# minyoungg/pix2latent

Measured on AMD Instinct MI355X. Metric: candidate-latent evals/sec (fwd+loss+bwd), BigGAN-256 pop=18, higher is better.
Workload: dtype f32 (fp32 tensors everywhere; convolutions >= 32x32 and the self-attention multiply on the 16-bit MFMA pipe with fp32-grade operand splits and fp32 accumulate: the 16x16 Winograd, direct and sub-pixel 3x3 kernels and the 1x1 kernels (4x4 layers included) on power-of-two scaled operands in 2 fp16 pie

## Files before the change

### include/p2l.h

```cpp
#ifndef P2L_H_
#define P2L_H_

#include <stddef.h>
#include <stdint.h>

#ifdef __cplusplus
extern "C" {
#endif

#define P2L_OK 0
#define P2L_EINVAL (-1)
#define P2L_ELAUNCH (-2)
#define P2L_EWS (-3)
#define P2L_EUNSUP (-4)

int p2l_version(void);
const char* p2l_strerror(int rc);
int p2l_last_hip_error(void);


enum { P2L_ACT_NONE = 0, P2L_ACT_RELU = 1, P2L_ACT_TANH = 2,
       P2L_ACT_LRELU_SQRT2 = 3  };
enum { P2L_POOL_NONE = 0, P2L_POOL_MAX = 1, P2L_POOL_SUM = 2 };
enum { P2L_PRO_NONE = 0, P2L_PRO_AFFINE_RELU = 1, P2L_PRO_AFFINE = 2 };
// ... 110 lines not shown
       P2L_WFMT_FLAG_ATTN_GEMM = 0x40,
       P2L_WFMT_FLAG_NO_AMAX = 0x80
                                       };
int p2l_pack_conv_weight_bf3t(const float* w_oihw, int O, int I, int N_pad, int K_pad,
                              int transpose_flip, float* w_packed, void* stream);
int p2l_pack_conv_weight_pw(const float* w_oihw, int O, int I, int N_pad, int K_pad,
                            int transpose_flip, float* w_packed, void* stream);
size_t p2l_packed_weight_floats(int taps, int N_pad, int K_pad, int wfmt);
enum {
  P2L_FORM_AUTO = 0,
  P2L_FORM_NO_WINO = 1,
  P2L_FORM_WINO_ANY = 2,
  P2L_FORM_WINO_8X16 = 4,
  P2L_FORM_NO_PW = 8,
  P2L_FORM_NO_THIN = 16,
  P2L_FORM_WINO_BF3 = 32,
  P2L_FORM_WINO_H2_8X16 = 64,
  P2L_FORM_WINO_H2_16X16 = 128,
  P2L_FORM_NO_H2R = 256,
  P2L_FORM_H2R_SEQ_EPI = 512,
  P2L_FORM_NO_SP_SKIP = 1024,
  P2L_FORM_NO_SP_PAIR = 2048,
  P2L_FORM_SP_PAIR = 4096,
  P2L_FORM_GENERIC_EPI = 8192
};
int p2l_conv_epilogue_class(const P2LConv* d, const P2LConvExtra* ex, const P2LArb* arb, const float* bias,
                            const float* res, const float* mask, const float* y, const float* yp,
                            const void* workspace, size_t ws_bytes);
int p2l_wino_split_factor(int H, int W, int Cin, int Cout);
int p2l_pack_conv_weight_bf3w(const float* w_oihw, int O, int I, int taps, int N_pad,
                              int K_pad, int transpose_flip, float* w_packed, void* stream);
int p2l_pack_conv_weight_bf3(const float* w_oihw, int O, int I, int taps, int N_pad,
                             int K_pad, int transpose_flip, float* w_packed, void* stream);
int p2l_pack_conv_weight_subpix_bf3(const float* w_oihw, int O, int I, int N_pad, int K_pad,
                                    int transpose_flip, int mode, float* w_packed,
                                    void* stream);
size_t p2l_packed_subpix_weight_floats(int N_pad, int K_pad, int wfmt);
int p2l_pack_conv_weight_subpix_h2(const float* w_oihw, int O, int I, int N_pad, int K_pad,
                                   int transpose_flip, int mode, float* w_packed, void* stream);

typedef struct P2LGemm {
  int32_t batch, M, N, K;
  int32_t lda, ldb, ldc;
  int64_t stride_a, stride_b, stride_c;
  int32_t a_kmajor, b_kmajor;
  float alpha;
  int32_t accumulate;
// ... 7 lines not shown
typedef struct P2LAttn {
  int32_t B, Nq, Nk, d, dv;
} P2LAttn;
int p2l_attn_supported(const P2LAttn* d);
size_t p2l_attn_fwd_ws_bytes(const P2LAttn* d);
int p2l_attn_fwd(const P2LAttn* d, const float* q, const float* k, const float* v, float* out,
                 float* lse, void* ws, size_t ws_bytes, void* stream);
size_t p2l_attn_bwd_dv_ws_bytes(const P2LAttn* d);
int p2l_attn_bwd_dv(const P2LAttn* d, const float* q, const float* k, const float* dout,
                    const float* lse, float* dv, void* ws, size_t ws_bytes, void* stream);
size_t p2l_attn_bwd_qk_ws_bytes(const P2LAttn* d);
int p2l_attn_bwd_qk(const P2LAttn* d, const float* q, const float* k, const float* v,
                    const float* out, const float* dout, const float* lse, float* dst, float* dq,
                    float* dk, void* ws, size_t ws_bytes, void* stream);

int p2l_linear_fwd(const float* x, const float* W, const float* bias, float* y,
                   int Bn, int K, int N, void* stream);
int p2l_linear_bwd(const float* dy, const float* W, float* dx, int Bn, int K,
                   int N, int accumulate, void* stream);
int p2l_linear_fwd_ld(const float* x, int x_ld, const float* W, const float* bias, float* y,
                      int Bn, int K, int N, void* stream);
int p2l_linear_bwd_ld(const float* dy, const float* W, float* dx, int dx_ld, int Bn, int K,
                      int N, int accumulate, void* stream);

int p2l_cbn_fold_fwd(const float* g_raw, const float* b_raw, const float* mean,
                     const float* rstd, float* s, float* t, int Bn, int C,
                     int raw_ld, void* stream);
int p2l_cbn_fold_bwd(const float* ds, const float* dt, const float* mean,
                     const float* rstd, float* dg_raw, float* db_raw, int Bn,
                     int C, int raw_ld, void* stream);

int p2l_affine_relu_bwd_nblk(int P);
int p2l_affine_relu_bwd(const float* da, int da_ld, const float* x, int x_ld,
                        const float* s, const float* t, int st_bstride,
                        const float* skip, int skip_ld, int skip_C, int skip_ups,
                        float* dx, int dx_ld, float* ds, float* dt,
                        int dsdt_bstride, float* partial, int Bn, int H, int W,
                        int C, void* stream);

int p2l_scale_bwd(const float* da, int da_ld, const float* x, int x_ld, const float* s,
                  int st_bstride, const float* skip, int skip_ld, int skip_C, float* dx,
                  int dx_ld, float* ds, float* dt_scratch, int dsdt_bstride, float* partial,
                  int Bn, int H, int W, int C, void* stream);

int p2l_softmax_fwd(const float* S, float* P, int64_t rows, int cols,
                    void* stream);
// ... 391 lines not shown
```

### pix2latent_amd/_native.py

```python
import ctypes as C
import os

import torch

_HERE = os.path.dirname(os.path.abspath(__file__))
LIB_PATH = os.environ.get('P2L_LIB_PATH') or os.path.join(_HERE, 'libp2l_hip.so')

c_float_p = C.c_void_p


class P2LConv(C.Structure):
    _fields_ = [('B', C.c_int32), ('H', C.c_int32), ('W', C.c_int32),
                ('Cin', C.c_int32), ('Cout', C.c_int32), ('taps', C.c_int32),
                ('ups', C.c_int32), ('x_ld', C.c_int32), ('pro', C.c_int32),
                ('pro_bstride', C.c_int32), ('alpha', C.c_float), ('act', C.c_int32),
                ('pool', C.c_int32), ('y_ld', C.c_int32), ('yp_ld', C.c_int32),
                ('n_store', C.c_int32), ('res_ld', C.c_int32), ('res_ups', C.c_int32),
                ('mask_ld', C.c_int32), ('splitk', C.c_int32), ('ext', C.c_int32),
                ('wfmt', C.c_int32), ('form', C.c_int32), ('algo_flops', C.c_double),
                ('w_floats', C.c_int64)]


class P2LAmax(C.Structure):
    _fields_ = [('out', C.c_void_p), ('outp', C.c_void_p), ('in_', C.c_void_p), ('in_n', C.c_int32),
# ... 123 lines not shown


def prof_totals():
    t = P2LProfTotals()
    t.size = C.sizeof(P2LProfTotals)
    check(lib().p2l_prof_totals(C.byref(t)), 'p2l_prof_totals')
    return t


prof_end = prof_totals


ACT_NONE, ACT_RELU, ACT_TANH, ACT_LRELU_SQRT2 = 0, 1, 2, 3
WFMT_F32, WFMT_BF16X3, WFMT_BF16X3W, WFMT_PW, WFMT_BF16X3T = 0, 1, 2, 3, 4
WFMT_FLAG_PW, WFMT_FLAG_THIN, WFMT_FLAG_ATTN_GEMM, WFMT_FLAG_NO_AMAX = 0x10, 0x20, 0x40, 0x80
FORM_AUTO, FORM_NO_WINO, FORM_WINO_ANY, FORM_WINO_8X16, FORM_NO_PW, FORM_NO_THIN, FORM_WINO_BF3 = 0, 1, 2, 4, 8, 16, 32
FORM_WINO_H2_8X16, FORM_WINO_H2_16X16 = 64, 128
FORM_H2R_SEQ_EPI = 512
FORM_NO_SP_SKIP = 1024
FORM_NO_SP_PAIR = 2048
FORM_SP_PAIR = 4096
FORM_NO_H2R = 256
FORM_GENERIC_EPI = 8192


def default_wfmt():
    v = os.environ.get('P2L_CONV_WFMT', 'bf16x3').lower()
    if v in ('f32', 'fp32', '0'):
        return WFMT_F32
    if v in ('bf16x3-direct', 'bf3d', '1'):
        return WFMT_BF16X3
    if v in ('bf16x3', 'bf3', 'bf16x3w', '2'):
        return WFMT_BF16X3W
    raise ValueError('P2L_CONV_WFMT=%r (expected f32, bf16x3 or bf16x3-direct)' % v)


def default_thin():
    return os.environ.get('P2L_THIN', '1') != '0' and default_wfmt() != WFMT_F32


def default_attn_gemm():
    return os.environ.get('P2L_ATTN', '1') == '0'


def default_no_amax():
    return os.environ.get('P2L_AMAX', '1') == '0'
# ... 45 lines not shown

POOL_NONE, POOL_MAX, POOL_SUM = 0, 1, 2
PRO_NONE, PRO_AFFINE_RELU, PRO_AFFINE = 0, 1, 2

EXPORTS = [
    'p2l_version', 'p2l_strerror', 'p2l_last_hip_error',
    'p2l_conv_workspace_bytes', 'p2l_conv_amax_slots', 'p2l_conv_epilogue_class', 'p2l_selftest_amaxreg', 'p2l_conv_suggest_splitk', 'p2l_conv_fwd', 'p2l_conv_fwd_ex',
    'p2l_pack_conv_weight', 'p2l_pack_conv_weight_subpix', 'p2l_pack_conv_weight_bf3',
    'p2l_pack_conv_weight_bf3w', 'p2l_packed_weight_floats', 
    'p2l_pack_conv_weight_bf3t',
    'p2l_pack_conv_weight_pw', 'p2l_adam_step_dev',
    'p2l_attn_supported', 'p2l_attn_fwd_ws_bytes', 'p2l_attn_fwd', 'p2l_attn_bwd_dv_ws_bytes',
    'p2l_attn_bwd_dv', 'p2l_attn_bwd_qk_ws_bytes', 'p2l_attn_bwd_qk',
    'p2l_pack_conv_weight_subpix_bf3', 'p2l_pack_conv_weight_subpix_h2', 'p2l_packed_subpix_weight_floats', 'p2l_gemm', 'p2l_gemm_ws_bytes', 'p2l_gemm_ws', 'p2l_linear_fwd', 'p2l_linear_bwd',
    'p2l_cbn_fold_fwd', 'p2l_cbn_fold_bwd', 'p2l_affine_relu_bwd_nblk',
    'p2l_affine_relu_bwd', 'p2l_softmax_fwd', 'p2l_softmax_bwd', 'p2l_maxpool2_bwd', 'p2l_maxpool2_bwd_amax', 'p2l_maxpool2_bwd_amax_slots',
    'p2l_relu_mask', 'p2l_nchw3_to_nhwc16', 'p2l_nhwc16_to_nchw3', 'p2l_tanh_bwd16',
    'p2l_weight_sum', 'p2l_weight_map', 'p2l_l1_loss_nblk', 'p2l_l1_loss_fwd',
    'p2l_l1_loss_bwd', 'p2l_lpips_normalize', 'p2l_lpips_tap_nblk', 'p2l_lpips_tap_fwd',
    'p2l_lpips_tap_bwd', 'p2l_lpips_tap_pool_bwd', 'p2l_bilinear_adjoint', 'p2l_reduce_rows', 'p2l_adam_step',
    'p2l_clamp', 'p2l_affine_grid_sample', 'p2l_affine_grid_sample_bwd', 'p2l_affine_grid_sample_bwd_ws_bytes', 'p2l_vec_scale_div', 'p2l_concat2', 'p2l_split2',
    'p2l_biggan_ws_bytes', 'p2l_biggan_fwd', 'p2l_biggan_bwd', 'p2l_biggan_ws_lookup',
    'p2l_loss_cache_floats', 'p2l_projloss_ws_bytes', 'p2l_projloss_ws_lookup', 'p2l_projloss_prepare',
    'p2l_projloss_fwd', 'p2l_projloss_bwd', 'p2l_mfma_probe', 'p2l_prof_begin', 'p2l_prof_totals', 'p2l_prof_step', 'p2l_prof_dump', 'p2l_wino_split_factor', 'p2l_linear_fwd_ld', 'p2l_linear_bwd_ld', 'p2l_scale_bwd',
    'p2l_sg2_pixelnorm_fwd', 'p2l_sg2_pixelnorm_bwd', 'p2l_sg2_bias_lrelu_fwd', 'p2l_sg2_lrelu_bwd',
    'p2l_sg2_demod_fwd', 'p2l_sg2_demod_bwd', 'p2l_sg2_blur_fwd', 'p2l_sg2_act_bwd_nblk',
    'p2l_sg2_styled_act_bwd', 'p2l_sg2_blur_bwd', 'p2l_sg2_rgb_up_fwd', 'p2l_sg2_rgb_up_bwd',
    'p2l_sg2_clamp16_fwd', 'p2l_sg2_clamp16_bwd', 'p2l_broadcast_rows', 'p2l_add_inplace',
    'p2l_sg2_ws_bytes', 'p2l_sg2_ws_lookup', 'p2l_sg2_synthesis_fwd', 'p2l_sg2_synthesis_bwd', 'p2l_sg2_mapping_fwd',
    'p2l_sg2_mapping_bwd', 'p2l_conv_arb_fusable', 'p2l_conv_arb_nblk',
    'p2l_conv_dgrad_arb', 'p2l_conv_arb_split_fusable', 'p2l_conv_arb_nblk_ws',
    'p2l_conv_dgrad_arb_ws', 'p2l_arb_finish', 'p2l_arb_defer_begin', 'p2l_arb_defer_flush',
    'p2l_arb_defer_cancel',
    'p2l_gconv_fwd', 'p2l_maxpool3s2_fwd', 'p2l_maxpool3s2_bwd', 'p2l_conv1_dgrad',
    'p2l_alex_cache_floats', 'p2l_alexloss_ws_bytes', 'p2l_alexloss_prepare', 'p2l_alexloss_fwd',
    'p2l_alexloss_bwd',
    'p2l_pack_gconv_weight', 'p2l_sqz_cache_floats', 'p2l_sqzloss_ws_bytes', 'p2l_sqzloss_prepare', 'p2l_sqzloss_fwd',
    'p2l_sqzloss_bwd', 'p2l_sqzloss_ws_lookup',
    'p2l_sg2_blur_fwd_amax', 'p2l_sg2_styled_act_bwd_amax', 'p2l_sg2_blur_bwd_amax', 'p2l_sg2_noise_relayout',
    'p2l_sg2_rows_defer_begin', 'p2l_sg2_rows_defer_flush', 'p2l_sg2_rows_defer_cancel',
    'p2l_color_adjust_ws_bytes', 'p2l_color_adjust',
    'p2l_gram_f64_ws_bytes', 'p2l_gram_f64', 'p2l_gram_f64_wide_ws_bytes', 'p2l_gram_f64_wide',
    'p2l_poisson_blend_ws_bytes', 'p2l_poisson_blend',
    'p2l_sg2_noise_reg_ws_bytes', 'p2l_sg2_noise_reg_fwd', 'p2l_sg2_noise_reg_bwd', 'p2l_sg2_noise_normalize',
    'p2l_area_pool3_to_nhwc16', 'p2l_area_pool_nchw', 'p2l_area_unpool16_add_nchw3',
    'p2l_latent_prior_ws_bytes', 'p2l_latent_prior_fwd', 'p2l_latent_prior_bwd',
    'p2l_l2_loss_nblk', 'p2l_l2_loss_fwd', 'p2l_l2_loss_bwd', 'p2l_adam_step_sched',
# ... 124 lines not shown
```

### pix2latent_amd/csrc/p2l_ops.hip

```cpp
#include "p2l_common.h"

namespace {

__device__ __forceinline__ float block_sum_256(float v, float* red ) {
  v = wave_sum(v);
  const int lane = threadIdx.x & 63, wave = threadIdx.x >> 6;
  __syncthreads();
  if (lane == 0) red[wave] = v;
  __syncthreads();
  return (red[0] + red[1]) + (red[2] + red[3]);
}

template <int BG>
__global__ __launch_bounds__(256) void linear_fwd_kernel(
    const float* __restrict__ x, const float* __restrict__ W,
    const float* __restrict__ bias, float* __restrict__ y, int Bn, int b_begin,
    int K, int N, int x_ld) {
  extern __shared__ float sm[];
  float* xs = sm;
  float* red = sm + BG * K;
  const int tid = threadIdx.x, nl = tid & 63, kg = tid >> 6;
  const int n = blockIdx.x * 64 + nl;
  const int nb = min(BG, Bn - b_begin);
  for (int i = tid; i < BG * K; i += 256) {
// ... 9 lines not shown
  if (n < N) {
#pragma unroll 8
    for (int kk = k0; kk < k0 + kper; ++kk) {
      const float w = W[(size_t)kk * N + n];
#pragma unroll
      for (int b = 0; b < BG; ++b) acc[b] = fmaf(xs[b * K + kk], w, acc[b]);
    }
  }
#pragma unroll
  for (int b = 0; b < BG; ++b) red[(kg * BG + b) * 64 + nl] = acc[b];
  __syncthreads();
  for (int i = tid; i < BG * 64; i += 256) {
    const int b = i >> 6, c = i & 63;
    const int nn = blockIdx.x * 64 + c;
    if (b < nb && nn < N) {
      float v = (red[(0 * BG + b) * 64 + c] + red[(1 * BG + b) * 64 + c]) +
                (red[(2 * BG + b) * 64 + c] + red[(3 * BG + b) * 64 + c]);
      if (bias) v += bias[nn];
      y[(size_t)(b_begin + b) * N + nn] = v;
    }
  }
}

template <int BG>
__global__ __launch_bounds__(1024) void linear_bwd_kernel(
    const float* __restrict__ dy, const float* __restrict__ W,
    float* __restrict__ dx, int Bn, int b_begin, int K, int N, int accumulate, int dx_ld) {
  __shared__ float red[BG][16];
  const int k = blockIdx.x, tid = threadIdx.x;
  const int nb = min(BG, Bn - b_begin);
  float acc[BG];
#pragma unroll
  for (int b = 0; b < BG; ++b) acc[b] = 0.f;
  const float* wrow = W + (size_t)k * N;
  const int N4 = N >> 2;
  for (int i = tid; i < N4; i += 1024) {
    const f32x4 w = *reinterpret_cast<const f32x4*>(wrow + 4 * i);
#pragma unroll
    for (int b = 0; b < BG; ++b) {
      if (b < nb) {
        const f32x4 d = *reinterpret_cast<const f32x4*>(dy + (size_t)(b_begin + b) * N + 4 * i);
        acc[b] += (d.x * w.x + d.y * w.y) + (d.z * w.z + d.w * w.w);
      }
    }
  }
  for (int n = 4 * N4 + tid; n < N; n += 1024) {
    const float w = wrow[n];
#pragma unroll
    for (int b = 0; b < BG; ++b)
      if (b < nb) acc[b] = fmaf(dy[(size_t)(b_begin + b) * N + n], w, acc[b]);
  }
  const int lane = tid & 63, wave = tid >> 6;
#pragma unroll
  for (int b = 0; b < BG; ++b) {
    const float v = wave_sum(acc[b]);
    if (lane == 0) red[b][wave] = v;
  }
  __syncthreads();
  if (tid < nb) {
    float s = 0.f;
#pragma unroll
    for (int w = 0; w < 16; ++w) s += red[tid][w];
    float* p = dx + (size_t)(b_begin + tid) * dx_ld + k;
    *p = accumulate ? (*p + s) : s;
  }
}

__global__ void cbn_fold_fwd_kernel(const float* g_raw, const float* b_raw,
                                    const float* mean, const float* rstd,
                                    float* s, float* t, int Bn, int C, int raw_ld) {
  const int i = blockIdx.x * 256 + threadIdx.x;
  if (i >= Bn * C) return;
  const int b = i / C, c = i - b * C;
  const float gain = 1.f + g_raw[(size_t)b * raw_ld + c];
  const float bias = b_raw[(size_t)b * raw_ld + c];
  const float sv = gain * rstd[c];
  s[i] = sv;
  t[i] = bias - mean[c] * sv;
}

__global__ void cbn_fold_bwd_kernel(const float* ds, const float* dt,
                                    const float* mean, const float* rstd,
                                    float* dg_raw, float* db_raw, int Bn, int C,
                                    int raw_ld) {
  const int i = blockIdx.x * 256 + threadIdx.x;
  if (i >= Bn * C) return;
// ... 797 lines not shown
  if (!x || !W || !y || K < 4 || K % 4 || K > 1024 || Bn < 1 || N < 1 || x_ld < K) return P2L_EINVAL;
  constexpr int BG = 16, BGW = 24;
  const size_t lds = (size_t)(BG * K + 4 * BG * 64) * sizeof(float);
  const size_t ldsw = (size_t)(BGW * K + 4 * BGW * 64) * sizeof(float);
  if (cdiv(Bn, BGW) < cdiv(Bn, BG) && ldsw <= 64 * 1024) {
    for (int b0 = 0; b0 < Bn; b0 += BGW)
      hipLaunchKernelGGL(linear_fwd_kernel<BGW>, dim3(cdiv(N, 64)), dim3(256), ldsw,
                         ST(stream), x, W, bias, y, Bn, b0, K, N, x_ld);
    return p2l_check_launch();
  }
  for (int b0 = 0; b0 < Bn; b0 += BG) {
    hipLaunchKernelGGL(linear_fwd_kernel<BG>, dim3(cdiv(N, 64)), dim3(256), lds,
                       ST(stream), x, W, bias, y, Bn, b0, K, N, x_ld);
  }
  return p2l_check_launch();
}

extern "C" int p2l_linear_bwd_ld(const float* dy, const float* W, float* dx, int dx_ld, int Bn,
                                 int K, int N, int accumulate, void* stream);
extern "C" int p2l_linear_bwd(const float* dy, const float* W, float* dx, int Bn,
                              int K, int N, int accumulate, void* stream) {
  return p2l_linear_bwd_ld(dy, W, dx, K, Bn, K, N, accumulate, stream);
}
extern "C" int p2l_linear_bwd_ld(const float* dy, const float* W, float* dx, int dx_ld, int Bn,
                                 int K, int N, int accumulate, void* stream) {
  if (!dy || !W || !dx || Bn < 1 || K < 1 || N < 4 || (N % 4) || dx_ld < K) return P2L_EINVAL;
  constexpr int BG = 16, BGW = 24;
  if (cdiv(Bn, BGW) < cdiv(Bn, BG)) {
    for (int b0 = 0; b0 < Bn; b0 += BGW)
      hipLaunchKernelGGL(linear_bwd_kernel<BGW>, dim3(K), dim3(1024), 0, ST(stream), dy,
                         W, dx, Bn, b0, K, N, accumulate, dx_ld);
    return p2l_check_launch();
  }
  for (int b0 = 0; b0 < Bn; b0 += BG)
    hipLaunchKernelGGL(linear_bwd_kernel<BG>, dim3(K), dim3(1024), 0, ST(stream), dy,
                       W, dx, Bn, b0, K, N, accumulate, dx_ld);
  return p2l_check_launch();
}

extern "C" int p2l_cbn_fold_fwd(const float* g_raw, const float* b_raw,
                                const float* mean, const float* rstd, float* s,
                                float* t, int Bn, int C, int raw_ld, void* stream) {
  if (!g_raw || !b_raw || !mean || !rstd || !s || !t) return P2L_EINVAL;
  if (Bn < 1 || C < 1 || raw_ld < C || (int64_t)Bn * C > INT32_MAX) return P2L_EINVAL;
  hipLaunchKernelGGL(cbn_fold_fwd_kernel, dim3(cdiv(Bn * C, 256)), dim3(256), 0,
                     ST(stream), g_raw, b_raw, mean, rstd, s, t, Bn, C, raw_ld);
  return p2l_check_launch();
}
extern "C" int p2l_cbn_fold_bwd(const float* ds, const float* dt, const float* mean,
                                const float* rstd, float* dg_raw, float* db_raw,
                                int Bn, int C, int raw_ld, void* stream) {
  if (!ds || !dt || !mean || !rstd || !dg_raw || !db_raw) return P2L_EINVAL;
  if (Bn < 1 || C < 1 || raw_ld < C || (int64_t)Bn * C > INT32_MAX) return P2L_EINVAL;
  hipLaunchKernelGGL(cbn_fold_bwd_kernel, dim3(cdiv(Bn * C, 256)), dim3(256), 0,
                     ST(stream), ds, dt, mean, rstd, dg_raw, db_raw, Bn, C, raw_ld);
  return p2l_check_launch();
}

extern "C" int p2l_affine_relu_bwd_nblk(int P) { return cdiv(P, ARB_SLAB); }

// ... 381 lines not shown
```

### pix2latent_amd/csrc/p2l_pw.hip

```cpp
#include "p2l_conv_k.h"
#include <type_traits>

#include <atomic>

using namespace p2lconv;

namespace {

template <int KS> struct PwCfg {
  static constexpr int SUB = KS / 16;
  static constexpr int A_FLOATS = SUB * 128 * 24;
  static constexpr int B_FLOATS = SUB * 64 * 24;
  static constexpr size_t LDS_BYTES = (size_t)(A_FLOATS + B_FLOATS) * sizeof(float);
};

__device__ __forceinline__ void pw_store_split(float* As, int row, int q4, const f32x4 x) {
  bf16x4 ph, pm, pl;
  split3(x, ph, pm, pl);
  char* rb = reinterpret_cast<char*>(As) + row * 96 + (q4 & 1) * 8;
  char* rq = rb + bf3_chunk(q4 >> 1, row) * 16;
  *reinterpret_cast<bf16x4*>(rq) = ph;
  *reinterpret_cast<bf16x4*>(rq + 32) = pm;
  *reinterpret_cast<bf16x4*>(rq + 64) = pl;
}
// ... 105 lines not shown
        f32x16 t = acc[j];
        t = __builtin_amdgcn_mfma_f32_32x32x16_bf16(a3, b1, t, 0, 0, 0);
        t = __builtin_amdgcn_mfma_f32_32x32x16_bf16(a1, b3, t, 0, 0, 0);
        t = __builtin_amdgcn_mfma_f32_32x32x16_bf16(a2, b2, t, 0, 0, 0);
        t = __builtin_amdgcn_mfma_f32_32x32x16_bf16(a2, b1, t, 0, 0, 0);
        t = __builtin_amdgcn_mfma_f32_32x32x16_bf16(a1, b2, t, 0, 0, 0);
        t = __builtin_amdgcn_mfma_f32_32x32x16_bf16(a1, b1, t, 0, 0, 0);
        acc[j] = t;
      }
    }
    __syncthreads();
    if (more) write_lds();
    __syncthreads();
  }
  epilogue_vec<2>(k, acc, smem, wave, lane, b0, y0, x0, n0, tile_in_image, 0, 0, 0);
}


constexpr int PWH_SUB = 2;
constexpr int PWH_A_FLOATS = PWH_SUB * 128 * 16, PWH_B_FLOATS = PWH_SUB * 64 * 16;
constexpr int PWH_EPI_FLOATS = 4 * 32 * (64 + 4);
constexpr size_t PWH_LDS_BYTES =
    (size_t)(PWH_A_FLOATS + PWH_B_FLOATS > PWH_EPI_FLOATS ? PWH_A_FLOATS + PWH_B_FLOATS : PWH_EPI_FLOATS) * sizeof(float);
__device__ __forceinline__ int h2_chunk(int c, int row) { return c ^ ((row >> 2) & 3); }
__device__ __forceinline__ int h2_chunk_a(int c, int row, int sub) { return h2_chunk(c, row) ^ ((sub & 1) << 1); }
__device__ __forceinline__ void pw_store_split_h2(float* As, int row, int q4, int sub, const f32x4 x) {
  const h16x4 h = __builtin_convertvector(x, h16x4);
  const f32x4 w = __builtin_convertvector(h, f32x4);
  const h16x4 m = __builtin_convertvector(x - w, h16x4);
  char* rb = reinterpret_cast<char*>(As) + row * 64 + (q4 & 1) * 8;
  *reinterpret_cast<h16x4*>(rb + h2_chunk_a(q4 >> 1, row, sub) * 16) = h;
  *reinterpret_cast<h16x4*>(rb + h2_chunk_a(2 + (q4 >> 1), row, sub) * 16) = m;
}

#ifndef P2L_PW_ABL
#define P2L_PW_ABL 0
#endif
template <int PRO, bool SM = false, int EC = EPI_GENERIC>
__global__ __launch_bounds__(256, SM ? 3 : 4) void pw_h2_kernel(const ConvK k) {
  static_assert(!SM || EC == EPI_GENERIC, "the small-grid form keeps the shared item");
  constexpr int KS = 32, VPP = KS / 4;
  constexpr int A_ITERS = 128 * VPP / 256;
  extern __shared__ __attribute__((aligned(16))) float smem[];
  float* As = smem;
  float* Bs = smem + PWH_A_FLOATS;
  float* scl = smem + PWH_LDS_BYTES / sizeof(float);

  const int tid = threadIdx.x;
  const int lane = tid & 63, wave = tid >> 6;
  const int l31 = lane & 31, lhi = lane >> 5;

  const int TW = 1 << k.tw_log, TH = 1 << k.th_log;
  const int swz = xcd_remap(blockIdx.x, gridDim.x);
  const int mt = swz / k.n_ntiles, nt = swz - mt * k.n_ntiles;
  const int tiles_per_image = k.tiles_x * k.tiles_y;
  const int bt = mt / tiles_per_image;
  const int b0 = SM ? (bt << k.tb_log) : bt;
  const int tile_in_image = mt - bt * tiles_per_image;
  const int ty = tile_in_image / k.tiles_x, tx = tile_in_image - ty * k.tiles_x;
  const int n0 = nt * 64;
  const int y0 = ty << k.th_log, x0 = tx << k.tw_log;

  float x_scale = 1.f, out_scale = 1.f;
// ... 39 lines not shown
                const f32x4 s4 = ps[c], t4 = pt[c];
                ms = fmaxf(fmaxf(ms, fmaxf(fabsf(s4.x), fabsf(s4.y))), fmaxf(fabsf(s4.z), fabsf(s4.w)));
                mt_ = fmaxf(fmaxf(mt_, fmaxf(fabsf(t4.x), fabsf(t4.y))), fmaxf(fabsf(t4.z), fabsf(t4.w)));
              }
            }
          } else {
            a = k.amax[b * 64 + lane];
          }
        }
#pragma unroll
        for (int o = 1; o < 64; o <<= 1) {
          a = fmaxf(a, __shfl_xor(a, o, 64));
          if (PRO != P2L_PRO_NONE) { ms = fmaxf(ms, __shfl_xor(ms, o, 64)); mt_ = fmaxf(mt_, __shfl_xor(mt_, o, 64)); }
        }
        if (PRO != P2L_PRO_NONE && k.amax_in != nullptr) a = (k.amax_in_applied ? a : ms * a + mt_) * 1.001f;
        float xs, inv_x;
        h2_scales(__builtin_bit_cast(unsigned, a), xs, inv_x);
        if (lane == 0) { scl[2 * t] = xs; scl[2 * t + 1] = inv_x * inv_w; }
      }
      __syncthreads();
    }
  }

  const int av = tid & (VPP - 1);
  int a_goff[A_ITERS], a_soff[SM ? A_ITERS : 1];
  float a_xs[SM ? A_ITERS : 1];
  unsigned a_valid = 0;
#pragma unroll
  for (int it = 0; it < A_ITERS; ++it) {
    const int p = (tid + 256 * it) / VPP;
    const int Q = p >> 2, s = p & 3;
    const int qx = Q & ((TW >> 1) - 1);
    const int qy = (Q >> (k.tw_log - 1)) & ((TH >> 1) - 1);
    const int iy = y0 + 2 * qy + (s >> 1), ix = x0 + 2 * qx + (s & 1);
    if (SM) {
      const int tb = Q >> (k.tw_log + k.th_log - 2);
      const int b = b0 + tb;
      a_goff[it] = 0; a_soff[it] = 0; a_xs[it] = scl[2 * tb];
      if (b < k.B) {
        a_goff[it] = ((b * k.H + iy) * k.W + ix) * k.x_ld + av * 4;
        a_soff[it] = b * k.pro_bstride + av * 4;
        a_valid |= 1u << it;
      }
    } else {
      a_goff[it] = ((b0 * k.H + iy) * k.W + ix) * k.x_ld + av * 4;
    }
  }
  const int s_off = b0 * k.pro_bstride + av * 4;
  constexpr int B_ITERS = PWH_SUB * 256 / 256;
  int b_goff[B_ITERS];
#pragma unroll
  for (int it = 0; it < B_ITERS; ++it) {
    const int j = tid + 256 * it;
    const int sub = j / 256, within = j - sub * 256;
    b_goff[it] = (sub * (k.Cout >> 5) + (n0 >> 5)) * 32 * 16 + within * 4;
  }
  const int b_stage = PWH_SUB * (k.Cout >> 5) * 32 * 16;

#ifdef P2L_AB_PW_SHALLOW
  constexpr bool DEEP = false;
#else
  constexpr bool DEEP = !SM;
#endif
  constexpr int NSET = DEEP ? 2 : 1;
  f32x4 xr[NSET][A_ITERS], wr[B_ITERS], sr[SM ? A_ITERS : 1], tr[SM ? A_ITERS : 1];
  __amdgpu_buffer_rsrc_t x_rs, w_rs;
  unsigned a_boff[A_ITERS], b_boff[B_ITERS];
  if (DEEP) {
    auto sgpr = [](const void* p) {
      const unsigned long long v = reinterpret_cast<unsigned long long>(p);
      const unsigned lo = __builtin_amdgcn_readfirstlane((unsigned)v);
      const unsigned hi = __builtin_amdgcn_readfirstlane((unsigned)(v >> 32));
      return reinterpret_cast<char*>(((unsigned long long)hi << 32) | lo);
    };
    const size_t img = (size_t)k.H * k.W * k.x_ld;
    x_rs = __builtin_amdgcn_make_buffer_rsrc(sgpr(k.x + (size_t)b0 * img), 0,
                                             __builtin_amdgcn_readfirstlane((int)(img * 4)), 0x00020000);
    w_rs = __builtin_amdgcn_make_buffer_rsrc(sgpr(k.w), 0,
                                             __builtin_amdgcn_readfirstlane(k.Cin * k.Cout * 4), 0x00020000);
#pragma unroll
    for (int it = 0; it < A_ITERS; ++it) a_boff[it] = (unsigned)(a_goff[it] - b0 * (int)img) * 4u;
#pragma unroll
    for (int it = 0; it < B_ITERS; ++it) b_boff[it] = (unsigned)b_goff[it] * 4u;
  }
  auto load_a = [&](int st, auto SET_) {
    constexpr int set = decltype(SET_)::value;
#pragma unroll
    for (int it = 0; it < A_ITERS; ++it) {
      if (DEEP) {
        xr[set][it] = __builtin_bit_cast(f32x4, __builtin_amdgcn_raw_buffer_load_b128(x_rs, a_boff[it], st * (KS * 4), 0));
        continue;
      }
      xr[set][it] = *reinterpret_cast<const f32x4*>(k.x + (size_t)a_goff[it] + st * KS);
      if (SM && PRO != P2L_PRO_NONE) {
        sr[it] = *reinterpret_cast<const f32x4*>(k.pro_s + a_soff[it] + st * KS);
        tr[it] = *reinterpret_cast<const f32x4*>(k.pro_t + a_soff[it] + st * KS);
      }
    }
  };
  float* st_lds = smem + PWH_LDS_BYTES / sizeof(float) + 32;
  auto load_b = [&](int st) {
    if (!SM && !DEEP && PRO != P2L_PRO_NONE) {
      sr[0] = *reinterpret_cast<const f32x4*>(k.pro_s + s_off + st * KS);
      tr[0] = *reinterpret_cast<const f32x4*>(k.pro_t + s_off + st * KS);
    }
#pragma unroll
    for (int it = 0; it < B_ITERS; ++it) {
      if (DEEP) wr[it] = __builtin_bit_cast(f32x4, __builtin_amdgcn_raw_buffer_load_b128(w_rs, b_boff[it], st * (b_stage * 4), 0));
      else wr[it] = *reinterpret_cast<const f32x4*>(k.w + (size_t)st * b_stage + b_goff[it]);
    }
  };
  auto write_lds = [&](auto SET_, int st) {
    constexpr int set = decltype(SET_)::value;
    if (!SM && DEEP && PRO != P2L_PRO_NONE) {
      sr[0] = *reinterpret_cast<const f32x4*>(st_lds + st * KS + av * 4);
      tr[0] = *reinterpret_cast<const f32x4*>(st_lds + k.Cin + st * KS + av * 4);
    }
#pragma unroll
    for (int it = 0; it < A_ITERS; ++it) {
      f32x4 v = xr[set][it];
      if (PRO != P2L_PRO_NONE) {
        v = v * sr[SM ? it : 0] + tr[SM ? it : 0];
        if (PRO == P2L_PRO_AFFINE_RELU) {
          v.x = fmaxf(v.x, 0.f); v.y = fmaxf(v.y, 0.f);
          v.z = fmaxf(v.z, 0.f); v.w = fmaxf(v.w, 0.f);
        }
      }
      if (SM && !((a_valid >> it) & 1u)) v = f32x4{0.f, 0.f, 0.f, 0.f};
      const int p = (tid + 256 * it) / VPP;
      pw_store_split_h2(As + (av >> 2) * (128 * 16), p, av & 3, av >> 2, v * (SM ? a_xs[it] : x_scale));
    }
#pragma unroll
    for (int it = 0; it < B_ITERS; ++it)
      *reinterpret_cast<f32x4*>(Bs + (tid + 256 * it) * 4) = wr[it];
  };

  f32x16 acc[2];
#pragma unroll
  for (int j = 0; j < 2; ++j)
#pragma unroll
    for (int r = 0; r < 16; ++r) acc[j][r] = 0.f;

  const int a_row = wave * 32 + l31;
  const int a_h = h2_chunk(lhi, a_row) * 4, a_m = h2_chunk(2 + lhi, a_row) * 4;
  const int b_h = h2_chunk(lhi, l31) * 4, b_m = h2_chunk(2 + lhi, l31) * 4;
  const int nstages = k.Cin / KS;
  const int st_lo = SM ? (int)blockIdx.y * k.chunks_per_split : 0;
  const int st_hi = SM ? min(nstages, st_lo + k.chunks_per_split) : nstages;
  using S0_ = std::integral_constant<int, 0>;
  using S1_ = std::integral_constant<int, NSET - 1>;
  auto stage = [&](int st, auto P_, auto Q_, auto FULL_) {
    constexpr bool full = decltype(FULL_)::value;
    const bool more = full || st + 1 < st_hi;
    if (DEEP) {
      if (more && !(P2L_PW_ABL & 2)) load_b(st + 1);
      if ((full || st + 2 < st_hi) && !(P2L_PW_ABL & 2)) load_a(st + 2, P_);
    } else if (more && !(P2L_PW_ABL & 2)) {
      load_a(st + 1, P_);
      load_b(st + 1);
    }
#pragma unroll
    for (int sub = 0; sub < PWH_SUB; ++sub) {
      const float* ar = As + (sub * 128 + a_row) * 16;
      const h16x8 ah = *reinterpret_cast<const h16x8*>(ar + ((sub & 1) ? a_m : a_h));
      const h16x8 am = *reinterpret_cast<const h16x8*>(ar + ((sub & 1) ? a_h : a_m));
#pragma unroll
      for (int j = 0; j < 2; ++j) {
        const float* br = Bs + (sub * 64 + j * 32 + l31) * 16;
        const h16x8 bh = *reinterpret_cast<const h16x8*>(br + b_h);
        const h16x8 bm = *reinterpret_cast<const h16x8*>(br + b_m);
        f32x16 t = acc[j];
        if (!(P2L_PW_ABL & 8)) {
        t = __builtin_amdgcn_mfma_f32_32x32x16_f16(am, bh, t, 0, 0, 0);
        t = __builtin_amdgcn_mfma_f32_32x32x16_f16(ah, bm, t, 0, 0, 0);
        t = __builtin_amdgcn_mfma_f32_32x32x16_f16(ah, bh, t, 0, 0, 0);
        } else { t[0] += (float)am[0] * (float)bh[0] + (float)ah[1] * (float)bm[1]; }
        acc[j] = t;
      }
    }
    if (!(P2L_PW_ABL & 16)) __syncthreads();
    if (more && !(P2L_PW_ABL & 1)) write_lds(Q_, st + 1);
    if (!(P2L_PW_ABL & 16)) __syncthreads();
  };
  load_a(st_lo, S0_{});
  load_b(st_lo);
  if (!SM && DEEP && PRO != P2L_PRO_NONE) {
    const float* ps = k.pro_s + (size_t)b0 * k.pro_bstride;
    const float* pt = k.pro_t + (size_t)b0 * k.pro_bstride;
    for (int c = tid * 4; c < k.Cin; c += 1024) {
      *reinterpret_cast<f32x4*>(st_lds + c) = *reinterpret_cast<const f32x4*>(ps + c);
      *reinterpret_cast<f32x4*>(st_lds + k.Cin + c) = *reinterpret_cast<const f32x4*>(pt + c);
    }
    __syncthreads();
  }
  write_lds(S0_{}, st_lo);
  if (DEEP && st_lo + 1 < st_hi) load_a(st_lo + 1, S1_{});
  __syncthreads();
  if (DEEP) {
    int st = st_lo;
    for (; st + 3 < st_hi; st += 2) {
      stage(st, S0_{}, S1_{}, std::true_type{});
      stage(st + 1, S1_{}, S0_{}, std::true_type{});
    }
    for (; st < st_hi; st += 2) {
      stage(st, S0_{}, S1_{}, std::false_type{});
      if (st + 1 < st_hi) stage(st + 1, S1_{}, S0_{}, std::false_type{});
    }
  } else {
    for (int st = st_lo; st < st_hi; ++st) stage(st, S0_{}, S0_{}, std::false_type{});
  }
  if (!SM) {
#pragma unroll
    for (int j = 0; j < 2; ++j)
#pragma unroll
// ... 85 lines not shown
  hipLaunchKernelGGL(pw_pack_h2_kernel, dim3(cdiv(total, 256)), dim3(256), 0, st, w_oihw, dst, O, I, N_pad,
                     K_pad, flip, tail);
  return p2l_check_launch();
}

int p2l_pw_epi_class(const ConvK& k, int pro) {
  if (k.amax_in == nullptr || k.amax != nullptr) return EPI_GENERIC;
  return epi_class_pw(k, pro);
}

int p2l_pw_launch(const ConvK& k, int pro, hipStream_t st) {
  dim3 grid(k.n_mtiles * k.n_ntiles), block(256);
#define P2L_PW(PRO)                                                                          \
  do {                                                                                       \
    static std::atomic<bool> attr_set{false};                                                \
    if (!attr_set) {                                                                         \
      (void)hipFuncSetAttribute((const void*)pw_bf3_kernel<PRO, 32>,                         \
                                hipFuncAttributeMaxDynamicSharedMemorySize, 160 * 1024);     \
      attr_set = true;                                                                       \
    }                                                                                        \
    hipLaunchKernelGGL((pw_bf3_kernel<PRO, 32>), grid, block, PwCfg<32>::LDS_BYTES, st, k);  \
  } while (0)
#define P2L_PWH(PRO, SMV) P2L_PWHE(PRO, SMV, EPI_GENERIC)
#define P2L_PWHE(PRO, SMV, ECV)                                                              \
  do {                                                                                       \
    static std::atomic<bool> attr_set{false};                                                \
    if (!attr_set) {                                                                         \
      (void)hipFuncSetAttribute((const void*)pw_h2_kernel<PRO, SMV, ECV>,                    \
                                hipFuncAttributeMaxDynamicSharedMemorySize, 160 * 1024);     \
      attr_set = true;                                                                       \
    }                                                                                        \
    hipLaunchKernelGGL((pw_h2_kernel<PRO, SMV, ECV>), gridh, block,                          \
                       PWH_LDS_BYTES + 128 + ((!SMV && PRO != P2L_PRO_NONE) ? (size_t)k.Cin * 8 : 0), st, k); \
  } while (0)
  if (k.amax_in != nullptr || k.amax != nullptr) {
    const bool sm = k.amax != nullptr;
    dim3 gridh(k.n_mtiles * k.n_ntiles, sm ? k.splitk : 1);
    if (sm) {
      if (pro == P2L_PRO_NONE) P2L_PWH(P2L_PRO_NONE, true);
      else if (pro == P2L_PRO_AFFINE_RELU) P2L_PWH(P2L_PRO_AFFINE_RELU, true);
      else P2L_PWH(P2L_PRO_AFFINE, true);
      return p2l_check_launch();
    }
    switch (p2l_pw_epi_class(k, pro)) {
      case EPI_BIAS_PS:       P2L_PWHE(P2L_PRO_AFFINE_RELU, false, EPI_BIAS_PS); break;
      case EPI_BIAS_RES_PS:   P2L_PWHE(P2L_PRO_AFFINE_RELU, false, EPI_BIAS_RES_PS); break;
      case EPI_BIAS_RESUP_PS: P2L_PWHE(P2L_PRO_AFFINE_RELU, false, EPI_BIAS_RESUP_PS); break;
      case EPI_ARB:           P2L_PWHE(P2L_PRO_NONE, false, EPI_ARB); break;
      case EPI_ARB_SKIP:      P2L_PWHE(P2L_PRO_NONE, false, EPI_ARB_SKIP); break;
      case EPI_ARB_SKIP_UP:   P2L_PWHE(P2L_PRO_NONE, false, EPI_ARB_SKIP_UP); break;
      default:
        if (pro == P2L_PRO_NONE) P2L_PWH(P2L_PRO_NONE, false);
        else if (pro == P2L_PRO_AFFINE_RELU) P2L_PWH(P2L_PRO_AFFINE_RELU, false);
        else P2L_PWH(P2L_PRO_AFFINE, false);
    }
    return p2l_check_launch();
  }
#undef P2L_PWH
#undef P2L_PWHE
  if (pro == P2L_PRO_NONE) P2L_PW(P2L_PRO_NONE);
  else if (pro == P2L_PRO_AFFINE_RELU) P2L_PW(P2L_PRO_AFFINE_RELU);
  else P2L_PW(P2L_PRO_AFFINE);
#undef P2L_PW
  return p2l_check_launch();
}
```

Baseline: 1222.

## Deep-pipeline small-grid pointwise conv and add multi-column linear backward kernel

The small-grid (split-K) pointwise fp16-split kernel now uses the double-buffered buffer-load pipeline. Per-sample prologue scale and shift vectors are staged once into LDS instead of being loaded per stage, with a fallback to the old shallow path when the vectors exceed a size cap or a form flag asks for it. Separately, linear backward gains a kernel that computes two or four output columns per block, reusing each dy load across columns, for large N. The deeper pipeline costs more registers and LDS, which may lower occupancy, and the new linear kernel changes reduction order.

Result: no change. 1217 (-0.3%).

```diff
diff --git a/include/p2l.h b/include/p2l.h
--- a/include/p2l.h
+++ b/include/p2l.h
@@ -156,7 +156,8 @@
   P2L_FORM_NO_SP_SKIP = 1024,
   P2L_FORM_NO_SP_PAIR = 2048,
   P2L_FORM_SP_PAIR = 4096,
-  P2L_FORM_GENERIC_EPI = 8192
+  P2L_FORM_GENERIC_EPI = 8192,
+  P2L_FORM_PW_SM_SHALLOW = 16384
 };
 int p2l_conv_epilogue_class(const P2LConv* d, const P2LConvExtra* ex, const P2LArb* arb, const float* bias,
                             const float* res, const float* mask, const float* y, const float* yp,
@@ -210,6 +211,8 @@
                       int Bn, int K, int N, void* stream);
 int p2l_linear_bwd_ld(const float* dy, const float* W, float* dx, int dx_ld, int Bn, int K,
                       int N, int accumulate, void* stream);
+int p2l_linear_bwd_cols(const float* dy, const float* W, float* dx, int dx_ld, int Bn, int K,
+                        int N, int accumulate, int cols, void* stream);
 
 int p2l_cbn_fold_fwd(const float* g_raw, const float* b_raw, const float* mean,
                      const float* rstd, float* s, float* t, int Bn, int C,
diff --git a/pix2latent_amd/_native.py b/pix2latent_amd/_native.py
--- a/pix2latent_amd/_native.py
+++ b/pix2latent_amd/_native.py
@@ -169,6 +169,7 @@
 FORM_SP_PAIR = 4096
 FORM_NO_H2R = 256
 FORM_GENERIC_EPI = 8192
+FORM_PW_SM_SHALLOW = 16384
 
 
 def default_wfmt():
@@ -260,7 +261,7 @@
     'p2l_clamp', 'p2l_affine_grid_sample', 'p2l_affine_grid_sample_bwd', 'p2l_affine_grid_sample_bwd_ws_bytes', 'p2l_vec_scale_div', 'p2l_concat2', 'p2l_split2',
     'p2l_biggan_ws_bytes', 'p2l_biggan_fwd', 'p2l_biggan_bwd', 'p2l_biggan_ws_lookup',
     'p2l_loss_cache_floats', 'p2l_projloss_ws_bytes', 'p2l_projloss_ws_lookup', 'p2l_projloss_prepare',
-    'p2l_projloss_fwd', 'p2l_projloss_bwd', 'p2l_mfma_probe', 'p2l_prof_begin', 'p2l_prof_totals', 'p2l_prof_step', 'p2l_prof_dump', 'p2l_wino_split_factor', 'p2l_linear_fwd_ld', 'p2l_linear_bwd_ld', 'p2l_scale_bwd',
+    'p2l_projloss_fwd', 'p2l_projloss_bwd', 'p2l_mfma_probe', 'p2l_prof_begin', 'p2l_prof_totals', 'p2l_prof_step', 'p2l_prof_dump', 'p2l_wino_split_factor', 'p2l_linear_fwd_ld', 'p2l_linear_bwd_ld', 'p2l_linear_bwd_cols', 'p2l_scale_bwd',
     'p2l_sg2_pixelnorm_fwd', 'p2l_sg2_pixelnorm_bwd', 'p2l_sg2_bias_lrelu_fwd', 'p2l_sg2_lrelu_bwd',
     'p2l_sg2_demod_fwd', 'p2l_sg2_demod_bwd', 'p2l_sg2_blur_fwd', 'p2l_sg2_act_bwd_nblk',
     'p2l_sg2_styled_act_bwd', 'p2l_sg2_blur_bwd', 'p2l_sg2_rgb_up_fwd', 'p2l_sg2_rgb_up_bwd',
diff --git a/pix2latent_amd/csrc/p2l_ops.hip b/pix2latent_amd/csrc/p2l_ops.hip
--- a/pix2latent_amd/csrc/p2l_ops.hip
+++ b/pix2latent_amd/csrc/p2l_ops.hip
@@ -55,6 +55,11 @@
   }
 }
 
+__device__ __forceinline__ float dot4_rounded(const f32x4 d, const f32x4 w) {
+#pragma clang fp contract(off)
+  return (d.x * w.x + d.y * w.y) + (d.z * w.z + d.w * w.w);
+}
+
 template <int BG>
 __global__ __launch_bounds__(1024) void linear_bwd_kernel(
     const float* __restrict__ dy, const float* __restrict__ W,
@@ -66,14 +71,14 @@
 #pragma unroll
   for (int b = 0; b < BG; ++b) acc[b] = 0.f;
   const float* wrow = W + (size_t)k * N;
-  const int N4 = N >> 2;
+  const int N4 = (N & 3) ? 0 : N >> 2;
   for (int i = tid; i < N4; i += 1024) {
     const f32x4 w = *reinterpret_cast<const f32x4*>(wrow + 4 * i);
 #pragma unroll
     for (int b = 0; b < BG; ++b) {
       if (b < nb) {
         const f32x4 d = *reinterpret_cast<const f32x4*>(dy + (size_t)(b_begin + b) * N + 4 * i);
-        acc[b] += (d.x * w.x + d.y * w.y) + (d.z * w.z + d.w * w.w);
+        acc[b] += dot4_rounded(d, w);
       }
     }
   }
@@ -95,6 +100,69 @@
 #pragma unroll
     for (int w = 0; w < 16; ++w) s += red[tid][w];
     float* p = dx + (size_t)(b_begin + tid) * dx_ld + k;
+    *p = accumulate ? (*p + s) : s;
+  }
+}
+
+template <int NB, int KB>
+__global__ __launch_bounds__(1024) void linear_bwd_cols_kernel(
+    const float* __restrict__ dy, const float* __restrict__ W,
+    float* __restrict__ dx, int nb, int b_begin, int K, int N, int accumulate, int dx_ld) {
+  __shared__ float red[NB][KB][16];
+  constexpr int G = NB * KB <= 32 ? NB : (NB % 8 == 0 && NB * KB <= 48) ? 8 : 4;
+  static_assert(NB % G == 0, "whole groups of rows");
+  const int k0 = blockIdx.x * KB, tid = threadIdx.x;
+  float acc[NB][KB];
+#pragma unroll
+  for (int b = 0; b < NB; ++b)
+#pragma unroll
+    for (int j = 0; j < KB; ++j) acc[b][j] = 0.f;
+  const float* wrow[KB];
+  const float* drow[NB];
+#pragma unroll
+  for (int j = 0; j < KB; ++j) wrow[j] = W + (size_t)min(k0 + j, K - 1) * N;
+#pragma unroll
+  for (int b = 0; b < NB; ++b) drow[b] = dy + (size_t)(b_begin + min(b, nb - 1)) * N;
+  const int N4 = (N & 3) ? 0 : N >> 2;
+  for (int i = tid; i < N4; i += 1024) {
+    f32x4 w[KB];
+#pragma unroll
+    for (int j = 0; j < KB; ++j) w[j] = *reinterpret_cast<const f32x4*>(wrow[j] + 4 * i);
+#pragma unroll
+    for (int g = 0; g < NB; g += G) {
+      f32x4 d[G];
+#pragma unroll
+      for (int b = 0; b < G; ++b) d[b] = *reinterpret_cast<const f32x4*>(drow[g + b] + 4 * i);
+#pragma unroll
+      for (int b = 0; b < G; ++b)
+#pragma unroll
+        for (int j = 0; j < KB; ++j)
+          acc[g + b][j] += dot4_rounded(d[b], w[j]);
+    }
+  }
+  for (int n = 4 * N4 + tid; n < N; n += 1024) {
+#pragma unroll
+    for (int b = 0; b < NB; ++b) {
+      const float d = drow[b][n];
+#pragma unroll
+      for (int j = 0; j < KB; ++j) acc[b][j] = fmaf(d, wrow[j][n], acc[b][j]);
+    }
+  }
+  const int lane = tid & 63, wave = tid >> 6;
+#pragma unroll
+  for (int b = 0; b < NB; ++b)
+#pragma unroll
+    for (int j = 0; j < KB; ++j) {
+      const float v = wave_sum(acc[b][j]);
+      if (lane == 0) red[b][j][wave] = v;
+    }
+  __syncthreads();
+  const int b = tid / KB, j = tid % KB;
+  if (b < nb && k0 + j < K) {
+    float s = 0.f;
+#pragma unroll
+    for (int w = 0; w < 16; ++w) s += red[b][j][w];
+    float* p = dx + (size_t)(b_begin + b) * dx_ld + k0 + j;
     *p = accumulate ? (*p + s) : s;
   }
 }
@@ -938,20 +1006,50 @@
                               int K, int N, int accumulate, void* stream) {
   return p2l_linear_bwd_ld(dy, W, dx, K, Bn, K, N, accumulate, stream);
 }
+namespace {
+constexpr int LINEAR_BWD_COLS_MIN_N = 32768;
+template <int KB>
+void linear_bwd_cols_pass(const float* dy, const float* W, float* dx, int dx_ld, int nb, int b0, int K, int N,
+                          int accumulate, void* stream) {
+#define P2L_LBC(NBV)                                                                                     \
+  hipLaunchKernelGGL((linear_bwd_cols_kernel<NBV, KB>), dim3(cdiv(K, KB)), dim3(1024), 0, ST(stream), dy, \
+                     W, dx, nb, b0, K, N, accumulate, dx_ld)
+  if (nb <= 4) P2L_LBC(4);
+  else if (nb <= 8) P2L_LBC(8);
+  else if (nb <= 12) P2L_LBC(12);
+  else if (nb <= 16 || KB > 2) P2L_LBC(16);
+  else if constexpr (KB <= 2) P2L_LBC(24);
+#undef P2L_LBC
+}
+}
+extern "C" int p2l_linear_bwd_cols(const float* dy, const float* W, float* dx, int dx_ld, int Bn,
+                                   int K, int N, int accumulate, int cols, void* stream) {
+  if (!dy || !W || !dx || Bn < 1 || K < 1 || N < 4 || dx_ld < K) return P2L_EINVAL;
+  if (cols != 0 && cols != 1 && cols != 2 && cols != 4) return P2L_EINVAL;
+  if (cols == 0) cols = N >= LINEAR_BWD_COLS_MIN_N ? 2 : 1;
+  constexpr int BG = 16, BGW = 24;
+  const int step = cdiv(Bn, BGW) < cdiv(Bn, BG) ? BGW : BG;
+  for (int b0 = 0; b0 < Bn; b0 += step) {
+    const int nb = Bn - b0 < step ? Bn - b0 : step;
+    if (cols == 1) {
+      if (step == BGW)
+        hipLaunchKernelGGL(linear_bwd_kernel<BGW>, dim3(K), dim3(1024), 0, ST(stream), dy,
+                           W, dx, Bn, b0, K, N, accumulate, dx_ld);
+      else
+        hipLaunchKernelGGL(linear_bwd_kernel<BG>, dim3(K), dim3(1024), 0, ST(stream), dy,
+                           W, dx, Bn, b0, K, N, accumulate, dx_ld);
+    } else if (cols == 4 && nb <= 16) {
+      linear_bwd_cols_pass<4>(dy, W, dx, dx_ld, nb, b0, K, N, accumulate, stream);
+    } else {
+      linear_bwd_cols_pass<2>(dy, W, dx, dx_ld, nb, b0, K, N, accumulate, stream);
+    }
+  }
+  return p2l_check_launch();
+}
 extern "C" int p2l_linear_bwd_ld(const float* dy, const float* W, float* dx, int dx_ld, int Bn,
                                  int K, int N, int accumulate, void* stream) {
-  if (!dy || !W || !dx || Bn < 1 || K < 1 || N < 4 || (N % 4) || dx_ld < K) return P2L_EINVAL;
-  constexpr int BG = 16, BGW = 24;
-  if (cdiv(Bn, BGW) < cdiv(Bn, BG)) {
-    for (int b0 = 0; b0 < Bn; b0 += BGW)
-      hipLaunchKernelGGL(linear_bwd_kernel<BGW>, dim3(K), dim3(1024), 0, ST(stream), dy,
-                         W, dx, Bn, b0, K, N, accumulate, dx_ld);
-    return p2l_check_launch();
-  }
-  for (int b0 = 0; b0 < Bn; b0 += BG)
-    hipLaunchKernelGGL(linear_bwd_kernel<BG>, dim3(K), dim3(1024), 0, ST(stream), dy,
-                       W, dx, Bn, b0, K, N, accumulate, dx_ld);
-  return p2l_check_launch();
+  if (N % 4) return P2L_EINVAL;
+  return p2l_linear_bwd_cols(dy, W, dx, dx_ld, Bn, K, N, accumulate, 0, stream);
 }
 
 extern "C" int p2l_cbn_fold_fwd(const float* g_raw, const float* b_raw,
diff --git a/pix2latent_amd/csrc/p2l_pw.hip b/pix2latent_amd/csrc/p2l_pw.hip
--- a/pix2latent_amd/csrc/p2l_pw.hip
+++ b/pix2latent_amd/csrc/p2l_pw.hip
@@ -151,6 +151,8 @@
 constexpr int PWH_EPI_FLOATS = 4 * 32 * (64 + 4);
 constexpr size_t PWH_LDS_BYTES =
     (size_t)(PWH_A_FLOATS + PWH_B_FLOATS > PWH_EPI_FLOATS ? PWH_A_FLOATS + PWH_B_FLOATS : PWH_EPI_FLOATS) * sizeof(float);
+constexpr size_t PWH_SM_VEC_BYTES = 16 * 1024;
+static_assert(PWH_LDS_BYTES + 128 + PWH_SM_VEC_BYTES <= 53 * 1024, "three small-grid blocks per CU");
 __device__ __forceinline__ int h2_chunk(int c, int row) { return c ^ ((row >> 2) & 3); }
 __device__ __forceinline__ int h2_chunk_a(int c, int row, int sub) { return h2_chunk(c, row) ^ ((sub & 1) << 1); }
 __device__ __forceinline__ void pw_store_split_h2(float* As, int row, int q4, int sub, const f32x4 x) {
@@ -165,9 +167,15 @@
 #ifndef P2L_PW_ABL
 #define P2L_PW_ABL 0
 #endif
-template <int PRO, bool SM = false, int EC = EPI_GENERIC>
+template <int PRO, bool SM = false, int EC = EPI_GENERIC, bool SHALLOW = false>
 __global__ __launch_bounds__(256, SM ? 3 : 4) void pw_h2_kernel(const ConvK k) {
   static_assert(!SM || EC == EPI_GENERIC, "the small-grid form keeps the shared item");
+  static_assert(SM || !SHALLOW, "the full-tile form has one pipeline");
+#ifdef P2L_AB_PW_SHALLOW
+  constexpr bool DEEP = false;
+#else
+  constexpr bool DEEP = !SHALLOW;
+#endif
   constexpr int KS = 32, VPP = KS / 4;
   constexpr int A_ITERS = 128 * VPP / 256;
   extern __shared__ __attribute__((aligned(16))) float smem[];
@@ -253,6 +261,11 @@
     }
   }
 
+  const int nstages = k.Cin / KS;
+  const int st_lo = SM ? (int)blockIdx.y * k.chunks_per_split : 0;
+  const int st_hi = SM ? min(nstages, st_lo + k.chunks_per_split) : nstages;
+  const int SC = (st_hi - st_lo) * KS;
+
   const int av = tid & (VPP - 1);
   int a_goff[A_ITERS], a_soff[SM ? A_ITERS : 1];
   float a_xs[SM ? A_ITERS : 1];
@@ -267,10 +280,11 @@
     if (SM) {
       const int tb = Q >> (k.tw_log + k.th_log - 2);
       const int b = b0 + tb;
-      a_goff[it] = 0; a_soff[it] = 0; a_xs[it] = scl[2 * tb];
+      a_goff[it] = 0; a_xs[it] = scl[2 * tb];
+      a_soff[it] = DEEP ? tb * 2 * SC + av * 4 : 0;
       if (b < k.B) {
         a_goff[it] = ((b * k.H + iy) * k.W + ix) * k.x_ld + av * 4;
-        a_soff[it] = b * k.pro_bstride + av * 4;
+        if (!DEEP) a_soff[it] = b * k.pro_bstride + av * 4;
         a_valid |= 1u << it;
       }
     } else {
@@ -288,13 +302,8 @@
   }
   const int b_stage = PWH_SUB * (k.Cout >> 5) * 32 * 16;
 
-#ifdef P2L_AB_PW_SHALLOW
-  constexpr bool DEEP = false;
-#else
-  constexpr bool DEEP = !SM;
-#endif
   constexpr int NSET = DEEP ? 2 : 1;
-  f32x4 xr[NSET][A_ITERS], wr[B_ITERS], sr[SM ? A_ITERS : 1], tr[SM ? A_ITERS : 1];
+  f32x4 xr[NSET][A_ITERS], wr[B_ITERS], sr[(SM && !DEEP) ? A_ITERS : 1], tr[(SM && !DEEP) ? A_ITERS : 1];
   __amdgpu_buffer_rsrc_t x_rs, w_rs;
   unsigned a_boff[A_ITERS], b_boff[B_ITERS];
   if (DEEP) {
@@ -305,12 +314,14 @@
       return reinterpret_cast<char*>(((unsigned long long)hi << 32) | lo);
     };
     const size_t img = (size_t)k.H * k.W * k.x_ld;
+    const int n_img = SM ? min(1 << k.tb_log, k.B - b0) : 1;
     x_rs = __builtin_amdgcn_make_buffer_rsrc(sgpr(k.x + (size_t)b0 * img), 0,
-                                             __builtin_amdgcn_readfirstlane((int)(img * 4)), 0x00020000);
+                                             __builtin_amdgcn_readfirstlane((int)(n_img * img * 4)), 0x00020000);
     w_rs = __builtin_amdgcn_make_buffer_rsrc(sgpr(k.w), 0,
                                              __builtin_amdgcn_readfirstlane(k.Cin * k.Cout * 4), 0x00020000);
 #pragma unroll
-    for (int it = 0; it < A_ITERS; ++it) a_boff[it] = (unsigned)(a_goff[it] - b0 * (int)img) * 4u;
+    for (int it = 0; it < A_ITERS; ++it)
+      a_boff[it] = (SM && !((a_valid >> it) & 1u)) ? 0u : (unsigned)(a_goff[it] - b0 * (int)img) * 4u;
 #pragma unroll
     for (int it = 0; it < B_ITERS; ++it) b_boff[it] = (unsigned)b_goff[it] * 4u;
   }
@@ -324,8 +335,8 @@
       }
       xr[set][it] = *reinterpret_cast<const f32x4*>(k.x + (size_t)a_goff[it] + st * KS);
       if (SM && PRO != P2L_PRO_NONE) {
-        sr[it] = *reinterpret_cast<const f32x4*>(k.pro_s + a_soff[it] + st * KS);
-        tr[it] = *reinterpret_cast<const f32x4*>(k.pro_t + a_soff[it] + st * KS);
+        sr[(SM && !DEEP) ? it : 0] = *reinterpret_cast<const f32x4*>(k.pro_s + a_soff[it] + st * KS);
+        tr[(SM && !DEEP) ? it : 0] = *reinterpret_cast<const f32x4*>(k.pro_t + a_soff[it] + st * KS);
       }
     }
   };
@@ -351,7 +362,13 @@
     for (int it = 0; it < A_ITERS; ++it) {
       f32x4 v = xr[set][it];
       if (PRO != P2L_PRO_NONE) {
-        v = v * sr[SM ? it : 0] + tr[SM ? it : 0];
+        f32x4 s4 = sr[(SM && !DEEP) ? it : 0], t4 = tr[(SM && !DEEP) ? it : 0];
+        if (SM && DEEP) {
+          const float* sp = st_lds + a_soff[it] + (st - st_lo) * KS;
+          s4 = *reinterpret_cast<const f32x4*>(sp);
+          t4 = *reinterpret_cast<const f32x4*>(sp + SC);
+        }
+        v = v * s4 + t4;
         if (PRO == P2L_PRO_AFFINE_RELU) {
           v.x = fmaxf(v.x, 0.f); v.y = fmaxf(v.y, 0.f);
           v.z = fmaxf(v.z, 0.f); v.w = fmaxf(v.w, 0.f);
@@ -375,9 +392,6 @@
   const int a_row = wave * 32 + l31;
   const int a_h = h2_chunk(lhi, a_row) * 4, a_m = h2_chunk(2 + lhi, a_row) * 4;
   const int b_h = h2_chunk(lhi, l31) * 4, b_m = h2_chunk(2 + lhi, l31) * 4;
-  const int nstages = k.Cin / KS;
-  const int st_lo = SM ? (int)blockIdx.y * k.chunks_per_split : 0;
-  const int st_hi = SM ? min(nstages, st_lo + k.chunks_per_split) : nstages;
   using S0_ = std::integral_constant<int, 0>;
   using S1_ = std::integral_constant<int, NSET - 1>;
   auto stage = [&](int st, auto P_, auto Q_, auto FULL_) {
@@ -421,6 +435,21 @@
     for (int c = tid * 4; c < k.Cin; c += 1024) {
       *reinterpret_cast<f32x4*>(st_lds + c) = *reinterpret_cast<const f32x4*>(ps + c);
       *reinterpret_cast<f32x4*>(st_lds + k.Cin + c) = *reinterpret_cast<const f32x4*>(pt + c);
+    }
+    __syncthreads();
+  }
+  if (SM && DEEP && PRO != P2L_PRO_NONE) {
+    const int SC4 = SC >> 2, n4 = SC4 << k.tb_log;
+    for (int i = tid; i < n4; i += 256) {
+      const int t = i / SC4, c = (i - t * SC4) * 4;
+      f32x4 s4 = f32x4{0.f, 0.f, 0.f, 0.f}, t4 = s4;
+      if (b0 + t < k.B) {
+        const size_t o = (size_t)(b0 + t) * k.pro_bstride + st_lo * KS + c;
+        s4 = *reinterpret_cast<const f32x4*>(k.pro_s + o);
+        t4 = *reinterpret_cast<const f32x4*>(k.pro_t + o);
+      }
+      *reinterpret_cast<f32x4*>(st_lds + t * 2 * SC + c) = s4;
+      *reinterpret_cast<f32x4*>(st_lds + t * 2 * SC + SC + c) = t4;
     }
     __syncthreads();
   }
@@ -552,24 +581,33 @@
     hipLaunchKernelGGL((pw_bf3_kernel<PRO, 32>), grid, block, PwCfg<32>::LDS_BYTES, st, k);  \
   } while (0)
 #define P2L_PWH(PRO, SMV) P2L_PWHE(PRO, SMV, EPI_GENERIC)
-#define P2L_PWHE(PRO, SMV, ECV)                                                              \
+#define P2L_PWHE(PRO, SMV, ECV) P2L_PWHS(PRO, SMV, ECV, false, (!SMV && PRO != P2L_PRO_NONE) ? (size_t)k.Cin * 8 : 0)
+#define P2L_PWHS(PRO, SMV, ECV, SHV, VEC_BYTES)                                              \
   do {                                                                                       \
     static std::atomic<bool> attr_set{false};                                                \
     if (!attr_set) {                                                                         \
-      (void)hipFuncSetAttribute((const void*)pw_h2_kernel<PRO, SMV, ECV>,                    \
+      (void)hipFuncSetAttribute((const void*)pw_h2_kernel<PRO, SMV, ECV, SHV>,               \
                                 hipFuncAttributeMaxDynamicSharedMemorySize, 160 * 1024);     \
       attr_set = true;                                                                       \
     }                                                                                        \
-    hipLaunchKernelGGL((pw_h2_kernel<PRO, SMV, ECV>), gridh, block,                          \
-                       PWH_LDS_BYTES + 128 + ((!SMV && PRO != P2L_PRO_NONE) ? (size_t)k.Cin * 8 : 0), st, k); \
+    hipLaunchKernelGGL((pw_h2_kernel<PRO, SMV, ECV, SHV>), gridh, block,                     \
+                       PWH_LDS_BYTES + 128 + (VEC_BYTES), st, k);                            \
   } while (0)
   if (k.amax_in != nullptr || k.amax != nullptr) {
     const bool sm = k.amax != nullptr;
     dim3 gridh(k.n_mtiles * k.n_ntiles, sm ? k.splitk : 1);
     if (sm) {
-      if (pro == P2L_PRO_NONE) P2L_PWH(P2L_PRO_NONE, true);
-      else if (pro == P2L_PRO_AFFINE_RELU) P2L_PWH(P2L_PRO_AFFINE_RELU, true);
-      else P2L_PWH(P2L_PRO_AFFINE, true);
+      const int slice_stages = k.chunks_per_split < k.Cin / 32 ? k.chunks_per_split : k.Cin / 32;
+      const size_t vec = pro == P2L_PRO_NONE ? 0 : ((size_t)slice_stages * 32 * 8) << k.tb_log;
+      if ((k.form & P2L_FORM_PW_SM_SHALLOW) || vec > PWH_SM_VEC_BYTES) {
+        if (pro == P2L_PRO_NONE) P2L_PWHS(P2L_PRO_NONE, true, EPI_GENERIC, true, 0);
+        else if (pro == P2L_PRO_AFFINE_RELU) P2L_PWHS(P2L_PRO_AFFINE_RELU, true, EPI_GENERIC, true, 0);
+        else P2L_PWHS(P2L_PRO_AFFINE, true, EPI_GENERIC, true, 0);
+      } else {
+        if (pro == P2L_PRO_NONE) P2L_PWHS(P2L_PRO_NONE, true, EPI_GENERIC, false, vec);
+        else if (pro == P2L_PRO_AFFINE_RELU) P2L_PWHS(P2L_PRO_AFFINE_RELU, true, EPI_GENERIC, false, vec);
+        else P2L_PWHS(P2L_PRO_AFFINE, true, EPI_GENERIC, false, vec);
+      }
       return p2l_check_launch();
     }
     switch (p2l_pw_epi_class(k, pro)) {
@@ -588,6 +626,7 @@
   }
 #undef P2L_PWH
 #undef P2L_PWHE
+#undef P2L_PWHS
   if (pro == P2L_PRO_NONE) P2L_PW(P2L_PRO_NONE);
   else if (pro == P2L_PRO_AFFINE_RELU) P2L_PW(P2L_PRO_AFFINE_RELU);
   else P2L_PW(P2L_PRO_AFFINE);
```
